# RQLuo/CDLNet-video

Measured on AMD Instinct MI355X. Metric: Mpix/s denoised (fwd+bwd) at K=30,M=64,P=7, higher is better.
Workload: dtype f32 (split-bf16 x3 MFMA, fp32 accumulate, fp32 storage)

## Files before the change

### cdlnet-video_amd/csrc/cdl_fused2d.hip

```cpp
#include <atomic>
#include <cstdlib>
#include <type_traits>
#include <mutex>
#include <utility>
#include <vector>

#include "cdl_common.h"
#include "cdl_fused_sweep.h"


namespace {

#include "cdl_wave_dev.h"

typedef __attribute__((ext_vector_type(4))) __bf16 bf16x4;

constexpr int WX = 2;
constexpr int RB = 8;
constexpr int TW = 32 * WX;
constexpr int HALO = 3;
constexpr int RTW = TW + 2 * HALO;
constexpr int RTC = RTW + 2;
constexpr int LDS_W = 32 * 64 * 16;
constexpr int LDS_TAU = 64 * 4;

constexpr int GW_TH = 16;
constexpr int GW_RTH = GW_TH + 2 * HALO;
constexpr int TROWS = GW_RTH + 1;
constexpr int TPITCH = 72;
constexpr int TCOPY = TROWS * TPITCH;
constexpr int WG_THIN_BYTES = 2 * 2 * 4 * TCOPY * 2;
constexpr int IMG_ELEMS = 32 * 32;

template <int WY_>
struct Shape {
    static_assert(WY_ == 2 || WY_ == 4, "64 x 16 or 64 x 32 tiles");
    static constexpr int WY = WY_;
    static constexpr int NW = WX * WY;
    static constexpr int NT = 64 * NW;
    static constexpr int TH = RB * WY;
    static constexpr int RTH = TH + 2 * HALO;
    static constexpr int PITCH = WY == 2 ? 28 : 44;
    static constexpr int COPY = RTC * PITCH;
    static constexpr int LDS_RT = 2 * 4 * COPY * 2;
    static constexpr int SLAB = RTH * RTW;
    static constexpr int LDS_RSUM = 4 * SLAB * 4;
    static constexpr int LDS_TACC = NW * 64 * 4;
    static constexpr int LDS_STAGE = LDS_RT + LDS_RSUM + LDS_W + LDS_TAU + LDS_TACC;
    static constexpr int LDS_DA_THIN = 2 * 4 * TCOPY * 2;
    static constexpr int LDS_DA = LDS_DA_THIN + NW * 2 * 2 * IMG_ELEMS * 2;
    static constexpr bool WREG = WY == 2;
};

struct FusedParams {
    const float *r;
    const float *zin;
    unsigned *map;
    float *zout;
    const float *tau;
    float *dtau;
    const uint4 *frags;
    float *patches;
    float sgn;
    int do_synth;
    CDL_DBG_FIELD(int dbg;)
    int N, H, W, tilesX, tilesY;
    int rev;
    const float *r2;
    float *da_partial;
    int drop_zout;
};
struct FusedMapParams : FusedParams {
    const float *cmap;
    const float *tslope;
    float *dtau_w;
    float *dcmap;
    int dc_add;
};

constexpr int MODE_MAP = 4, MODE_FWD_MAP = MODE_FWD | MODE_MAP, MODE_FIRST_MAP = MODE_FIRST | MODE_MAP, MODE_BWD_MAP = MODE_BWD | MODE_MAP;
template <int MODE_M> using StageParams = std::conditional_t<(MODE_M & MODE_MAP) != 0, FusedMapParams, FusedParams>;

__device__ __forceinline__ float embed7(const float *w, int P, int i, int j)
{
    const int off = (7 - P) / 2;
    const int ii = i - off, jj = j - off;
    if (i > 6 || j > 6 || ii < 0 || jj < 0 || ii >= P || jj >= P) return 0.0f;
    return w[ii * P + jj];
}

__device__ __forceinline__ void prep_one(const float *__restrict__ wA, const float *__restrict__ wB,
                                         uint4 *__restrict__ out, int MT, int P, int t)
{
    const int FA = MT * 4, FB = 4 * MT;
    if (t >= (FA + FB) * 64) return;
    const int lane = t & 63, f = t >> 6;
    const int row = lane & 31, h = lane >> 5;
    const int PP = P * P;
    float v[8];
    if (f < FA) {
        const int R = f / 4, ks = f % 4;
        const int ch = 32 * R + row;
#pragma unroll
        for (int jj = 0; jj < 8; ++jj) v[jj] = embed7(wA + (size_t)ch * PP, P, jj, 2 * ks + h);
    } else {
        const int g = f - FA;
        const int Rp = g / (2 * MT), ksB = g % (2 * MT);
        const int R = ksB >> 1, s = ksB & 1;
        const int tap = 32 * Rp + row;
#pragma unroll
        for (int jj = 0; jj < 8; ++jj) {
            const int ch = 32 * R + 16 * s + 8 * (jj >> 2) + 4 * h + (jj & 3);
            v[jj] = embed7(wB + (size_t)ch * PP, P, tap >> 3, tap & 7);
        }
    }
    bf16x8 hi, lo;
#pragma unroll
    for (int jj = 0; jj < 8; ++jj) {
        __bf16 hh, ll;
        split_bf16(v[jj], hh, ll);
        hi[jj] = hh;
        lo[jj] = ll;
    }
    uint4 *hi_dst, *lo_dst;
    if (f < FA) { hi_dst = out + (size_t)f * 64; lo_dst = out + (size_t)(FA + f) * 64; }
    else { hi_dst = out + (size_t)(2 * FA + (f - FA)) * 64; lo_dst = out + (size_t)(2 * FA + FB + (f - FA)) * 64; }
    hi_dst[lane] = __builtin_bit_cast(uint4, hi);
    lo_dst[lane] = __builtin_bit_cast(uint4, lo);
}

__global__ void k_prep(const float *__restrict__ wA, const float *__restrict__ wB,
                       uint4 *__restrict__ out, int MT, int P)
{
    prep_one(wA, wB, out, MT, P, blockIdx.x * blockDim.x + threadIdx.x);
}

constexpr int PREP_BATCH = 32;
struct PrepBatch {
    const float *wA[PREP_BATCH];
    const float *wB[PREP_BATCH];
};
__global__ void k_prep_batch(PrepBatch b, uint4 *__restrict__ out, int frag_uint4, int MT, int P)
{
    prep_one(b.wA[blockIdx.y], b.wB[blockIdx.y], out + (size_t)blockIdx.y * frag_uint4, MT, P,
             blockIdx.x * blockDim.x + threadIdx.x);
}

#ifndef CDL_POL_STAGE_FAT_LD
#define CDL_POL_STAGE_FAT_LD 2
#endif
#ifndef CDL_POL_STAGE_FAT_ST
#define CDL_POL_STAGE_FAT_ST 0
#endif
#ifndef CDL_POL_WGRAD_FAT_LD
#define CDL_POL_WGRAD_FAT_LD 2
#endif
struct CachePolicy {
    static constexpr int stage_fat_ld = CDL_POL_STAGE_FAT_LD;
    static constexpr int stage_fat_st = CDL_POL_STAGE_FAT_ST;
    static constexpr int wgrad_fat_ld = CDL_POL_WGRAD_FAT_LD;
    static constexpr int narrow = 0;
};
__device__ __forceinline__ __amdgpu_buffer_rsrc_t fat_rsrc(const float *base, size_t img_floats)
{
    return __builtin_amdgcn_make_buffer_rsrc(const_cast<float *>(base), 0, (int)(img_floats * 4), 0x00020000);
}
__device__ __forceinline__ float buf_ld(__amdgpu_buffer_rsrc_t r, int voff, int soff)
{
    return __builtin_bit_cast(float, __builtin_amdgcn_raw_buffer_load_b32(r, voff, soff, CachePolicy::narrow));
}
__device__ __forceinline__ void buf_st(float v, __amdgpu_buffer_rsrc_t r, int voff, int soff)
{
    __builtin_amdgcn_raw_buffer_store_b32(__builtin_bit_cast(unsigned, v), r, voff, soff, CachePolicy::narrow);
}

enum { LAY_NCHW = 0, LAY_BLK = 1, LAY_BLK16 = 2 };
typedef __attribute__((ext_vector_type(2))) unsigned u32x2;

__host__ __device__ inline size_t blk_image_elems(int M, int H, int W) { return (size_t)H * ((W + 31) / 32) * M * 32; }
template <int LAY> __host__ __device__ inline size_t lay_image_bytes(int M, int H, int W)
{
    return LAY == LAY_NCHW ? (size_t)M * H * W * 4 : blk_image_elems(M, H, W) * (LAY == LAY_BLK ? 4 : 2);
}


__device__ __forceinline__ float bf16_round(float v) { return (float)(__bf16)v; }

template <int MT>
__device__ __forceinline__ void blk16_load_raw(u32x2 (&z)[MT][4], __amdgpu_buffer_rsrc_t rs, int voff)
{
#pragma unroll
    for (int R = 0; R < MT; ++R)
#pragma unroll
        for (int q = 0; q < 4; ++q)
            z[R][q] = __builtin_bit_cast(u32x2, __builtin_amdgcn_raw_buffer_load_b64(rs, voff, (8 * R + 2 * q) * 32 * 8, CachePolicy::narrow));
}
__device__ __forceinline__ float blk16_decode(const u32x2 &u, int e)
{
    const unsigned w = (e & 2) ? u.y : u.x;
    return __builtin_bit_cast(float, (e & 1) ? (w & 0xffff0000u) : (w << 16));
}

template <int LAY, int MT, int POL>
__device__ __forceinline__ void blk_load(float (&z)[MT][16], __amdgpu_buffer_rsrc_t rs, int voff)
{
    constexpr int EB = LAY == LAY_BLK ? 16 : 8;
#pragma unroll
    for (int R = 0; R < MT; ++R)
#pragma unroll
        for (int q = 0; q < 4; ++q) {
            const int soff = (8 * R + 2 * q) * 32 * EB;
            if constexpr (LAY == LAY_BLK) {
                typedef __attribute__((ext_vector_type(4))) float f32x4;
                const f32x4 f = __builtin_bit_cast(f32x4, __builtin_amdgcn_raw_buffer_load_b128(rs, voff, soff, POL));
                z[R][4 * q + 0] = f.x; z[R][4 * q + 1] = f.y; z[R][4 * q + 2] = f.z; z[R][4 * q + 3] = f.w;
            } else {
                const u32x2 u = __builtin_bit_cast(u32x2, __builtin_amdgcn_raw_buffer_load_b64(rs, voff, soff, CachePolicy::narrow));
                z[R][4 * q + 0] = __builtin_bit_cast(float, u.x << 16);
                z[R][4 * q + 1] = __builtin_bit_cast(float, u.x & 0xffff0000u);
                z[R][4 * q + 2] = __builtin_bit_cast(float, u.y << 16);
                z[R][4 * q + 3] = __builtin_bit_cast(float, u.y & 0xffff0000u);
            }
        }
}
template <int LAY, int POL>
__device__ __forceinline__ void blk_store4(float a0, float a1, float a2, float a3, __amdgpu_buffer_rsrc_t rs, int voff, int quad_pair)
{
    constexpr int EB = LAY == LAY_BLK ? 16 : 8;
    const int soff = quad_pair * 32 * EB;
    if constexpr (LAY == LAY_BLK) {
        typedef __attribute__((ext_vector_type(4))) float f32x4;
        const f32x4 f = {a0, a1, a2, a3};
        __builtin_amdgcn_raw_buffer_store_b128(__builtin_bit_cast(u32x4, f), rs, voff + soff, 0, POL);
    } else {
        u32x2 u;
        u.x = (__builtin_bit_cast(unsigned, a0) >> 16) | (__builtin_bit_cast(unsigned, a1) & 0xffff0000u);
        u.y = (__builtin_bit_cast(unsigned, a2) >> 16) | (__builtin_bit_cast(unsigned, a3) & 0xffff0000u);
        __builtin_amdgcn_raw_buffer_store_b64(u, rs, voff, soff, CachePolicy::narrow);
    }
}

template <int N>
__device__ __forceinline__ float lane_transpose_sum(const float (&v)[N], int c)
{
    float r = LaneTransposeSum<N>::run(v, c);
    if (N == 16) r += __shfl_xor(r, 16, 64);
    return r;
}

__device__ __forceinline__ float col2im_row(const float (&rv)[4], int h)
{
    const float r4 = upper_half_to_lower(rv[0]);
    const float r5 = upper_half_to_lower(rv[1]);
    const float r6 = upper_half_to_lower(rv[2]);
    const bool lo = h == 0;
    float s = lo ? r6 : 0.0f;
    s = wave_shr1(s) + (lo ? r5 : 0.0f);
    s = wave_shr1(s) + (lo ? r4 : 0.0f);
    s = wave_shr1(s) + (lo ? rv[3] : 0.0f);
    s = wave_shr1(s) + (lo ? rv[2] : 0.0f);
    s = wave_shr1(s) + (lo ? rv[1] : 0.0f);
    s = wave_shr1(s) + (lo ? rv[0] : 0.0f);
    return s;
}

constexpr int RUN = 8;
typedef __attribute__((ext_vector_type(2))) __bf16 bf16x2;
template <int S>
__device__ __forceinline__ void store_run(__bf16 *dst, const __bf16 (&v)[RUN], bool low)
{
    static_assert(S >= 0 && S <= 3, "four shifted copies");
    if (!low) {
        if constexpr (S == 1) dst[-1] = v[0];
        if constexpr (S == 2) *reinterpret_cast<bf16x2 *>(dst - 2) = bf16x2{v[0], v[1]};
        if constexpr (S == 3) { dst[-3] = v[0]; *reinterpret_cast<bf16x2 *>(dst - 2) = bf16x2{v[1], v[2]}; }
    }
    *reinterpret_cast<bf16x4 *>(dst) = bf16x4{v[S], v[S + 1], v[S + 2], v[S + 3]};
    if constexpr (S == 0) *reinterpret_cast<bf16x4 *>(dst + 4) = bf16x4{v[4], v[5], v[6], v[7]};
    if constexpr (S == 1) { *reinterpret_cast<bf16x2 *>(dst + 4) = bf16x2{v[5], v[6]}; dst[6] = v[7]; }
    if constexpr (S == 2) *reinterpret_cast<bf16x2 *>(dst + 4) = bf16x2{v[6], v[7]};
    if constexpr (S == 3) dst[4] = v[7];
}
template <int PREC>
__device__ __forceinline__ void store_run_copies(__bf16 *dst, int copy_elems, const float (&f)[RUN], bool low)
{
    __bf16 hh[RUN], ll[RUN];
#pragma unroll
    for (int j = 0; j < RUN; ++j) split_bf16(f[j], hh[j], ll[j]);
    store_run<0>(dst, hh, low); store_run<1>(dst + copy_elems, hh, low);
    store_run<2>(dst + 2 * copy_elems, hh, low); store_run<3>(dst + 3 * copy_elems, hh, low);
    if (PREC != 1) {
        dst += 4 * copy_elems;
        store_run<0>(dst, ll, low); store_run<1>(dst + copy_elems, ll, low);
        store_run<2>(dst + 2 * copy_elems, ll, low); store_run<3>(dst + 3 * copy_elems, ll, low);
    }
}


struct TileAt { int tile, n, tyi, txi; };
__device__ __forceinline__ TileAt tile_decode(int t, int numTiles, int tilesX, int tilesY, int rev)
{
    TileAt q;
    q.tile = rev ? numTiles - 1 - t : t;
    int bid = q.tile;
    q.txi = bid % tilesX; bid /= tilesX;
    q.tyi = bid % tilesY;
    q.n = bid / tilesY;
    return q;
}

__device__ __forceinline__ bf16x8 lds_window8(const __bf16 *p)
{
    const bf16x4 a0 = *reinterpret_cast<const bf16x4 *>(p);
    const bf16x4 a1 = *reinterpret_cast<const bf16x4 *>(p + 4);
    return __builtin_shufflevector(a0, a1, 0, 1, 2, 3, 4, 5, 6, 7);
}

template <int N>
__device__ __forceinline__ void zero_tiles(f32x16 (&a)[N])
{
#pragma unroll
    for (int i = 0; i < N; ++i)
#pragma unroll
        for (int v = 0; v < 16; ++v) a[i][v] = 0.0f;
}

__device__ __forceinline__ float4 lane_channel_quad(const float *src, int R, int qv, int h)
{
    return *reinterpret_cast<const float4 *>(&src[32 * R + 8 * qv + 4 * h]);
}
template <int MT>
__device__ __forceinline__ void lane_channel_values(float (&out)[MT * 16], const float *src, int h)
{
#pragma unroll
    for (int R = 0; R < MT; ++R)
#pragma unroll
        for (int qv = 0; qv < 4; ++qv) {
            const float4 s4 = lane_channel_quad(src, R, qv, h);
            out[16 * R + 4 * qv + 0] = s4.x; out[16 * R + 4 * qv + 1] = s4.y;
            out[16 * R + 4 * qv + 2] = s4.z; out[16 * R + 4 * qv + 3] = s4.w;
        }
}

template <bool ALO>
__device__ __forceinline__ void wgrad_transpose_store(__bf16 *img, int qv, int c, int h, bf16x4 hi4, bf16x4 lo4)
{
    const int slot = (2 * qv + h) ^ ((c >> 1) & 7);
    __bf16 *dst = img + c * 32 + slot * 4;
    *reinterpret_cast<bf16x4 *>(dst) = hi4;
    if (ALO) *reinterpret_cast<bf16x4 *>(dst + IMG_ELEMS) = lo4;
}
template <bool ALO>
__device__ __forceinline__ void wgrad_transpose_store(__bf16 *img, int qv, int c, int h, float v0, float v1, float v2, float v3)
{
    const float val[4] = {v0, v1, v2, v3};
    bf16x4 hi4, lo4;
#pragma unroll
    for (int e = 0; e < 4; ++e) {
        __bf16 hh, ll;
        split_bf16(val[e], hh, ll);
        hi4[e] = hh;
        lo4[e] = ll;
    }
    wgrad_transpose_store<ALO>(img, qv, c, h, hi4, lo4);
}

template <int MT, int PREC, bool ALO>
__device__ __forceinline__ void wgrad_products(f32x16 (&acc)[MT][2], const __bf16 *wimg, const __bf16 *thin_hi, int yl,
                                               int wxi, int lane)
{
    const int c = lane & 31, h = lane >> 5;
#pragma unroll
    for (int kk = 0; kk < 2; ++kk) {
        bf16x8 Bh[2], Bl[2];
#pragma unroll
        for (int tt = 0; tt < 2; ++tt) {
            const int tap = 32 * tt + c, ti = tap >> 3, tj = tap & 7;
            const int e0 = wxi * 32 + 16 * kk + 8 * h + (tj & 4);
            const __bf16 *ph = thin_hi + (tj & 3) * TCOPY + (yl + ti) * TPITCH + e0;
            Bh[tt] = lds_window8(ph);
            if (PREC != 1) Bl[tt] = lds_window8(ph + 4 * TCOPY);
        }
#pragma unroll
        for (int R = 0; R < MT; ++R) {
            const int gg = (lane >> 4) & 1, qq = (lane >> 2) & 3, pp = lane & 3;
            bf16x4 part[2][2];
#pragma unroll
            for (int half = 0; half < 2; ++half) {
                const int row = 16 * kk + 8 * h + 4 * half + qq;
                const int slot = (4 * gg + pp) ^ ((row >> 1) & 7);
                const __bf16 *src = wimg + (size_t)(R * 2) * IMG_ELEMS + row * 32 + slot * 4;
                part[0][half] = __builtin_amdgcn_ds_read_tr16_b64_v4bf16(
                    (__attribute__((address_space(3))) bf16x4 *)(src));
                if (ALO)
                    part[1][half] = __builtin_amdgcn_ds_read_tr16_b64_v4bf16(
                        (__attribute__((address_space(3))) bf16x4 *)(src + IMG_ELEMS));
            }
            const bf16x8 Ah = __builtin_shufflevector(part[0][0], part[0][1], 0, 1, 2, 3, 4, 5, 6, 7);
// ... 56 lines not shown
    constexpr bool MAP = (MODE_M & MODE_MAP) != 0;
    using G = Shape<WY>;
    constexpr int NW = G::NW, NT = G::NT, TH = G::TH, RTH = G::RTH, PITCH = G::PITCH, COPY = G::COPY, SLAB = G::SLAB;
    constexpr int LDS_RT = G::LDS_RT, LDS_RSUM = G::LDS_RSUM, LDS_STAGE = G::LDS_STAGE, LDS_DA_THIN = G::LDS_DA_THIN;
    static_assert(!DA || (MODE == MODE_BWD && TH == GW_TH), "dA_k rides in the reverse stage, on k_wgrad2d's 64 x 16 tiles");
    extern __shared__ __attribute__((aligned(16))) unsigned char smem[];
    __bf16 *rt = reinterpret_cast<__bf16 *>(smem);
    float *rsum_all = reinterpret_cast<float *>(smem + LDS_RT);
    const uint4 *wl = reinterpret_cast<const uint4 *>(smem + LDS_RT + LDS_RSUM);
    float *tau_s = reinterpret_cast<float *>(smem + LDS_RT + LDS_RSUM + LDS_W);
    float *tacc_s = tau_s + 64;
    __bf16 *thin2 = reinterpret_cast<__bf16 *>(smem + LDS_STAGE);
    __bf16 *imgs2 = reinterpret_cast<__bf16 *>(smem + LDS_STAGE + LDS_DA_THIN);
    float *slope_s = MODE == MODE_BWD ? tau_s : tacc_s;
    float *tacc_w_s = reinterpret_cast<float *>(smem + LDS_STAGE + (DA ? G::LDS_DA : 0));

    constexpr int M = 32 * MT;
    constexpr int FA = MT * 4, FB = 4 * MT;
    constexpr int NFRAG = (PREC != 1 ? 2 : 1) * (FA + FB);
    const int tid = threadIdx.x, lane = tid & 63, wid = tid >> 6;
    const int wxi = wid % WX, wyi = wid / WX;
    const int c = lane & 31, h = lane >> 5;
    const size_t HW = (size_t)p.H * p.W;
    const int numTiles = p.N * p.tilesY * p.tilesX;

    {
        uint4 *z4 = reinterpret_cast<uint4 *>(smem);
        for (int i = tid; i < (LDS_RT + LDS_RSUM) / 16; i += NT) z4[i] = make_uint4(0, 0, 0, 0);
        uint4 *wdst = reinterpret_cast<uint4 *>(smem + LDS_RT + LDS_RSUM);
        if (PREC != 1) {
            for (int i = tid; i < NFRAG * 64; i += NT) wdst[i] = p.frags[i];
        } else {
            for (int i = tid; i < FA * 64; i += NT) wdst[i] = p.frags[i];
            for (int i = tid; i < FB * 64; i += NT) wdst[FA * 64 + i] = p.frags[2 * FA * 64 + i];
        }
        if constexpr (MAP) {
            if (tid < M) slope_s[tid] = p.tslope[tid];
        }
    }
    constexpr int RT_RUNS = (RTH + RUN - 1) / RUN;
    static_assert(RTW * RT_RUNS <= NT && RT_RUNS * RUN <= PITCH, "one run per thread; a column's runs stay inside its pitch");
    const int rt_xx = tid % RTW, rt_y0 = (tid / RTW) * RUN;
    const bool rt_on = tid < RTW * RT_RUNS;
    __bf16 *const rt_dst = rt + rt_xx * PITCH + rt_y0;
    float stg[RUN];
    auto stage_load = [&](int t) {
        const TileAt q = tile_decode(t, numTiles, p.tilesX, p.tilesY, p.rev);
        const float *rimg = p.r + (size_t)q.n * HW;
        const int gy0 = q.tyi * TH - HALO + rt_y0, gx = q.txi * TW - HALO + rt_xx;
        const bool colok = rt_on && t < numTiles && !CDL_DBG(p.dbg, 8) && gx >= 0 && gx < p.W;
#pragma unroll
        for (int j = 0; j < RUN; ++j) {
            const int gy = gy0 + j;
            float v = 0.0f;
            if (colok && rt_y0 + j < RTH && gy >= 0 && gy < p.H) v = rimg[(size_t)gy * p.W + gx];
            stg[j] = v;
        }
    };
    auto stage_store = [&]() {
        if (rt_on) store_run_copies<PREC>(rt_dst, COPY, stg, rt_y0 == 0);
    };
    constexpr int T2_RUNS = (RTW + RUN - 1) / RUN;
    static_assert(!DA || (GW_RTH * T2_RUNS <= NT && T2_RUNS * RUN <= TPITCH), "one run per thread; a row's runs stay inside its pitch");
    const int t2_x0 = (tid % T2_RUNS) * RUN, t2_yy = tid / T2_RUNS;
    const bool t2_on = tid < GW_RTH * T2_RUNS;
    __bf16 *const t2_dst = thin2 + t2_yy * TPITCH + t2_x0;
    float stg2[DA ? RUN : 1];
    auto stage2_load = [&](int t) {
        const TileAt q = tile_decode(t, numTiles, p.tilesX, p.tilesY, p.rev);
        const float *timg = p.r2 + (t < numTiles ? (size_t)q.n * HW : 0);
        const int gy = q.tyi * TH - HALO + t2_yy, gx0 = q.txi * TW - HALO + t2_x0;
        const bool rowok = t2_on && t < numTiles && !CDL_DBG(p.dbg, 8) && gy >= 0 && gy < p.H;
#pragma unroll
        for (int j = 0; j < (DA ? RUN : 1); ++j) {
            const int gx = gx0 + j;
            const bool ok = rowok && t2_x0 + j < RTW && gx >= 0 && gx < p.W;
            const float v = timg[ok ? (size_t)gy * p.W + gx : 0];
            stg2[j] = ok ? v : 0.0f;
        }
    };
    auto stage2_store = [&]() {
        if constexpr (DA) {
            if (t2_on) store_run_copies<PREC>(t2_dst, TCOPY, stg2, t2_x0 == 0);
        }
    };
    f32x16 dacc[DA ? MT : 1][2];
    if constexpr (DA) {
#pragma unroll
        for (int R = 0; R < MT; ++R) zero_tiles(dacc[R]);
        for (int i = tid; i < LDS_DA_THIN / 16; i += NT) reinterpret_cast<uint4 *>(thin2)[i] = make_uint4(0, 0, 0, 0);
        stage2_load(blockIdx.x);
    }
    stage_load(blockIdx.x);
    __syncthreads();
    stage_store();
    if constexpr (DA) stage2_store();

    constexpr int OFF_AH = 0;
    constexpr int OFF_AL = FA;
    constexpr int OFF_BH = (PREC != 1 ? 2 * FA : FA);
    constexpr int OFF_BL = 2 * FA + FB;
    constexpr bool WREG = G::WREG;
    bf16x8 wreg[WREG ? NFRAG : 1];
    if constexpr (WREG) {
#pragma unroll
        for (int f = 0; f < NFRAG; ++f) wreg[f] = __builtin_bit_cast(bf16x8, wl[f * 64 + lane]);
    }
    auto wfrag = [&](int f) __attribute__((always_inline)) {
        if constexpr (WREG) return wreg[f];
        else return __builtin_bit_cast(bf16x8, wl[f * 64 + lane]);
    };

    constexpr bool MAP_FWD = MAP && MODE != MODE_BWD;
    float tslr[MAP_FWD ? MT * 16 : 1];
    bool slope_any = false;
    if constexpr (MAP_FWD) {
        lane_channel_values<MT>(tslr, slope_s, h);
        slope_any = __ballot(lane < M && !(slope_s[lane] >= 0.0f && slope_s[lane] < __builtin_inff())) != 0ull;
    }

    const int xl = wxi * 32 + c;
    float *rsum = rsum_all + ((wxi & 1) + 2 * (wyi & 1)) * SLAB;
    const bool has_base = (MODE == MODE_FWD) || (MODE == MODE_BWD && p.zin != nullptr);
    const int hw4 = (int)HW * 4;

#pragma unroll 1
    for (int t = blockIdx.x; t < numTiles; t += gridDim.x) {
    const TileAt at = tile_decode(t, numTiles, p.tilesX, p.tilesY, p.rev);
    const int tile = at.tile, n = at.n;
    const int tx0 = at.txi * TW, ty0 = at.tyi * TH;
    const int x = tx0 + xl;
    if (MODE != MODE_BWD && tid < M) tau_s[tid] = p.tau[(size_t)n * M + tid];
    __syncthreads();
    constexpr bool LOAD_AHEAD = MODE != MODE_BWD || WY == 2;
    if (LOAD_AHEAD) {
        stage_load(t + gridDim.x);
        if constexpr (DA) stage2_load(t + gridDim.x);
    }

    float ring[7][4];
#pragma unroll
    for (int i = 0; i < 7; ++i)
#pragma unroll
        for (int j = 0; j < 4; ++j) ring[i][j] = 0.0f;
    float tsum[MT * 16];
#pragma unroll
    for (int i = 0; i < MT * 16; ++i) tsum[i] = 0.0f;
    constexpr bool MAP_BWD = MAP && MODE == MODE_BWD;
    float tsum_w[MAP_BWD ? MT * 16 : 1];
    if constexpr (MAP_BWD) {
#pragma unroll
        for (int i = 0; i < MT * 16; ++i) tsum_w[i] = 0.0f;
    }
    const bool tau_neg = (MODE != MODE_BWD && __ballot(lane < M && !(tau_s[lane] >= 0.0f)) != 0ull) || slope_any;
    float taur[MT * 16];
    if (MODE != MODE_BWD) lane_channel_values<MT>(taur, tau_s, h);

    const bool xok = x < p.W;
    const size_t img_in = lay_image_bytes<LIN>(M, p.H, p.W), img_out = lay_image_bytes<LOUT>(M, p.H, p.W);
    const __amdgpu_buffer_rsrc_t rs_in = uniform_rsrc(
        has_base ? (const char *)p.zin + (size_t)n * img_in : (const char *)p.zout, has_base ? img_in : 0);
    unsigned *const map_n = p.map ? p.map + ((size_t)n * 4 + 2 * h) * HW : nullptr;
    const __amdgpu_buffer_rsrc_t rs_out = uniform_rsrc((const char *)p.zout + (size_t)n * img_out, img_out);
    const int lane_off = (int)((4 * h) * HW + x) * 4;
    const int XB = (p.W + 31) / 32, xb = (tx0 >> 5) + wxi;
    constexpr int EB_IN = LIN == LAY_BLK16 ? 8 : 16, EB_OUT = LOUT == LAY_BLK16 ? 8 : 16;
    const int lane_blk_in = (h * 32 + c) * EB_IN, lane_blk_out = (h * 32 + c) * EB_OUT;

#pragma unroll 1
    for (int b = 0; b < RB; ++b) {
        const int yl = wyi * RB + b;
        const int y = ty0 + yl;
        const bool valid = xok && (y < p.H);
        const int voff = valid ? lane_off + y * p.W * 4 : OOB;
        const int blk = (y * XB + xb) * (M / 4) * 32;
        const int voff_in = LIN == LAY_NCHW ? voff : (valid ? blk * EB_IN + lane_blk_in : OOB);
        const int voff_st = (CDL_DBG(p.dbg, 1) || (MODE == MODE_BWD && p.drop_zout)) ? OOB : (LOUT == LAY_NCHW ? voff : (valid ? blk * EB_OUT + lane_blk_out : OOB));

        float zc[MT][16];
        u32x2 zr[MT][4];
        if (MODE != MODE_FIRST && LIN == LAY_BLK16) {
            blk16_load_raw<MT>(zr, rs_in, voff_in);
        } else if (MODE != MODE_FIRST && CDL_DBG(p.dbg, 16)) {
#pragma unroll
            for (int R = 0; R < MT; ++R)
#pragma unroll
                for (int v = 0; v < 16; ++v) zc[R][v] = 0.25f;
        } else if (MODE != MODE_FIRST && LIN != LAY_NCHW) {
            blk_load<LIN, MT, CachePolicy::stage_fat_ld>(zc, rs_in, voff_in);
        } else if (MODE != MODE_FIRST) {
#pragma unroll
            for (int R = 0; R < MT; ++R)
#pragma unroll
                for (int v = 0; v < 16; ++v) {
                    const int soff = (32 * R + 8 * (v >> 2) + (v & 3)) * hw4;
                    zc[R][v] = buf_ld(rs_in, voff, soff);
                }
        }
        unsigned sup = 0, sgb = 0;
        if (MODE == MODE_BWD && valid) {
            sup = map_n[(size_t)y * p.W + x];
            sgb = map_n[HW + (size_t)y * p.W + x];
        }
        float cm = 0.0f;
        if constexpr (MAP) {
            if (valid) cm = p.cmap[(size_t)n * HW + (size_t)y * p.W + x];
        }

        const int q = b & 3, e = yl - q;
        bf16x8 rh[4], rl[4];
#pragma unroll
        for (int ks = 0; ks < 4; ++ks) {
            const int col = xl + 2 * ks + h;
            rh[ks] = lds_window8(rt + (0 * 4 + q) * COPY + col * PITCH + e);
            if (PREC != 1) rl[ks] = lds_window8(rt + (1 * 4 + q) * COPY + col * PITCH + e);
        }

        __builtin_amdgcn_sched_barrier(0);
        f32x16 acc[MT];
        zero_tiles(acc);
        if CDL_DBG(p.dbg, 4) {
#pragma unroll
            for (int R = 0; R < MT; ++R) acc[R][0] = (float)rh[0][0] + (float)rl[1][1];
        } else {
            bf16x8 wh[2][MT], wlo[2][MT];
#pragma unroll
            for (int R = 0; R < MT; ++R) {
                wh[0][R] = wfrag(OFF_AH + R * 4);
                if (PREC != 1) wlo[0][R] = wfrag(OFF_AL + R * 4);
            }
#pragma unroll
            for (int ks = 0; ks < 4; ++ks) {
                const int cu = ks & 1, nx = cu ^ 1;
                if (ks + 1 < 4) {
#pragma unroll
                    for (int R = 0; R < MT; ++R) {
                        wh[nx][R] = wfrag(OFF_AH + R * 4 + ks + 1);
                        if (PREC != 1) wlo[nx][R] = wfrag(OFF_AL + R * 4 + ks + 1);
                    }
                }
                if (PREC != 1) {
#pragma unroll
                    for (int R = 0; R < MT; ++R) acc[R] = __builtin_amdgcn_mfma_f32_32x32x16_bf16(wlo[cu][R], rh[ks], acc[R], 0, 0, 0);
#pragma unroll
                    for (int R = 0; R < MT; ++R) acc[R] = __builtin_amdgcn_mfma_f32_32x32x16_bf16(wh[cu][R], rl[ks], acc[R], 0, 0, 0);
                    if (PREC == 2) {
#pragma unroll
                        for (int R = 0; R < MT; ++R) acc[R] = __builtin_amdgcn_mfma_f32_32x32x16_bf16(wlo[cu][R], rl[ks], acc[R], 0, 0, 0);
                    }
                }
#pragma unroll
                for (int R = 0; R < MT; ++R) acc[R] = __builtin_amdgcn_mfma_f32_32x32x16_bf16(wh[cu][R], rh[ks], acc[R], 0, 0, 0);
            }
        }

        __builtin_amdgcn_sched_barrier(0);
        auto epilogue = [&](auto general_shrink) {
#pragma unroll
        for (int R = 0; R < MT; ++R)
#pragma unroll
            for (int v = 0; v < 16; ++v) {
                const int chl = 32 * R + 8 * (v >> 2) + (v & 3);
                float zz;
                float zbase = 0.0f;
                if (MODE != MODE_FIRST) zbase = LIN == LAY_BLK16 ? blk16_decode(zr[R][v >> 2], v & 3) : zc[R][v];
                if (MODE == MODE_BWD) {
                    const bool on = (sup >> (16 * R + v)) & 1u;
                    zz = on ? zbase + acc[R][v] : 0.0f;
                    const float gt = ((sgb >> (16 * R + v)) & 1u) ? zz : -zz;
                    tsum[16 * R + v] += gt;
                    if constexpr (MAP_BWD) tsum_w[16 * R + v] = fmaf(cm, gt, tsum_w[16 * R + v]);
                } else {
                    const float base = (MODE == MODE_FWD) ? zbase : 0.0f;
                    const float u = fmaf(p.sgn, acc[R][v], base);
                    float tt = taur[16 * R + v];
                    if constexpr (MAP_FWD) tt = cdl_map_threshold(tt, cm, tslr[16 * R + v]);
                    const float st = decltype(general_shrink)::value ? cdl_shrink(u, tt)
                                                                     : u - __builtin_amdgcn_fmed3f(u, -tt, tt);
                    zz = CDL_DBG(p.dbg, 64) ? u : (valid ? st : 0.0f);
                }
                if (LOUT == LAY_BLK16) zz = bf16_round(zz);
                if (LOUT == LAY_NCHW) buf_st(zz, rs_out, voff_st, chl * hw4);
                acc[R][v] = zz;
            }
        };
        bool general = tau_neg;
        if constexpr (MAP_FWD) general = general || __ballot(!(cm >= 0.0f && cm < __builtin_inff())) != 0ull;
        if (general) epilogue(std::true_type{});
        else epilogue(std::false_type{});
        if (LOUT != LAY_NCHW) {
#pragma unroll
            for (int R = 0; R < MT; ++R)
#pragma unroll
                for (int q = 0; q < 4; ++q)
                    blk_store4<LOUT, CachePolicy::stage_fat_st>(acc[R][4 * q], acc[R][4 * q + 1], acc[R][4 * q + 2], acc[R][4 * q + 3], rs_out,
                                     voff_st, 8 * R + 2 * q);
        }
        if (MODE != MODE_BWD && map_n) {
            unsigned ws = 0, wg = 0;
#pragma unroll
            for (int R = 0; R < MT; ++R)
#pragma unroll
                for (int v = 0; v < 16; ++v) {
                    const float zz = acc[R][v];
                    ws |= (zz != 0.0f ? 1u : 0u) << (16 * R + v);
                    wg |= (__builtin_bit_cast(unsigned, zz) >> 31) << (16 * R + v);
                }
            if (valid && !CDL_DBG(p.dbg, 1)) {
                map_n[(size_t)y * p.W + x] = ws;
                map_n[HW + (size_t)y * p.W + x] = wg;
            }
        }
        if constexpr (MAP_BWD) {
            if (p.dcmap) {
                float dcs = 0.0f;
#pragma unroll
                for (int R = 0; R < MT; ++R)
#pragma unroll
                    for (int qv = 0; qv < 4; ++qv) {
                        const float4 s4 = lane_channel_quad(slope_s, R, qv, h);
                        const float sl[4] = {s4.x, s4.y, s4.z, s4.w};
#pragma unroll
                        for (int e = 0; e < 4; ++e) {
                            const int v = 4 * qv + e;
                            const float zz = acc[R][v];
                            dcs = fmaf(sl[e], ((sgb >> (16 * R + v)) & 1u) ? zz : -zz, dcs);
                        }
                    }
                dcs += __shfl_xor(dcs, 32, 64);
                if (h == 0 && valid) {
                    float *dst = p.dcmap + (size_t)n * HW + (size_t)y * p.W + x;
                    *dst = p.dc_add ? *dst + dcs : dcs;
                }
            }
        }
        if constexpr (DA) {
            __bf16 *wimg = imgs2 + (size_t)wid * (MT * 2) * IMG_ELEMS;
            constexpr bool ALO = PREC != 1 && LOUT != LAY_BLK16;
#pragma unroll
            for (int R = 0; R < MT; ++R)
#pragma unroll
                for (int qv = 0; qv < 4; ++qv)
                    wgrad_transpose_store<ALO>(wimg + (size_t)(R * 2) * IMG_ELEMS, qv, c, h, acc[R][4 * qv], acc[R][4 * qv + 1],
                                               acc[R][4 * qv + 2], acc[R][4 * qv + 3]);
            __builtin_amdgcn_fence(__ATOMIC_RELEASE, "wavefront");
            __builtin_amdgcn_wave_barrier();
            wgrad_products<MT, PREC, ALO>(dacc, wimg, thin2, yl, wxi, lane);
        }
        if (MODE == MODE_BWD && !p.do_synth) continue;
        if CDL_DBG(p.dbg, 2) { ring[0][0] += acc[0][0] + acc[MT - 1][15]; continue; }

        __builtin_amdgcn_sched_barrier(0);
        f32x16 D[2];
        zero_tiles(D);
        {
            bf16x8 bwh[2][2], bwl[2][2];
#pragma unroll
            for (int Rp = 0; Rp < 2; ++Rp) {
                bwh[0][Rp] = wfrag(OFF_BH + Rp * 2 * MT);
                if (PREC != 1) bwl[0][Rp] = wfrag(OFF_BL + Rp * 2 * MT);
            }
#pragma unroll
            for (int q = 0; q < 2 * MT; ++q) {
                const int R = q >> 1, s = q & 1, cu = q & 1, nx = cu ^ 1;
                if (q + 1 < 2 * MT) {
#pragma unroll
                    for (int Rp = 0; Rp < 2; ++Rp) {
                        bwh[nx][Rp] = wfrag(OFF_BH + Rp * 2 * MT + q + 1);
                        if (PREC != 1) bwl[nx][Rp] = wfrag(OFF_BL + Rp * 2 * MT + q + 1);
                    }
                }
                bf16x8 zh, zl;
#pragma unroll
                for (int jj = 0; jj < 8; ++jj) {
                    __bf16 hh, ll;
                    split_bf16(acc[R][8 * s + jj], hh, ll);
                    zh[jj] = hh;
                    if (PREC != 1 && LOUT != LAY_BLK16) zl[jj] = ll;
                }
                if (PREC != 1) {
#pragma unroll
                    for (int Rp = 0; Rp < 2; ++Rp) D[Rp] = __builtin_amdgcn_mfma_f32_32x32x16_bf16(bwl[cu][Rp], zh, D[Rp], 0, 0, 0);
                    if (LOUT != LAY_BLK16) {
#pragma unroll
                        for (int Rp = 0; Rp < 2; ++Rp) D[Rp] = __builtin_amdgcn_mfma_f32_32x32x16_bf16(bwh[cu][Rp], zl, D[Rp], 0, 0, 0);
                        if (PREC == 2) {
#pragma unroll
                            for (int Rp = 0; Rp < 2; ++Rp) D[Rp] = __builtin_amdgcn_mfma_f32_32x32x16_bf16(bwl[cu][Rp], zl, D[Rp], 0, 0, 0);
                        }
                    }
                }
#pragma unroll
                for (int Rp = 0; Rp < 2; ++Rp) D[Rp] = __builtin_amdgcn_mfma_f32_32x32x16_bf16(bwh[cu][Rp], zh, D[Rp], 0, 0, 0);
            }
        }

        __builtin_amdgcn_sched_barrier(0);
#pragma unroll
        for (int Rp = 0; Rp < 2; ++Rp)
#pragma unroll
            for (int v = 0; v < 16; ++v) {
                const int i = 4 * Rp + (v >> 2);
                if (i <= 6) ring[i][v & 3] += D[Rp][v];
            }
        {
            const float cs = col2im_row(ring[0], h);
            if (lane < 38 && !CDL_DBG(p.dbg, 32)) rsum[yl * RTW + 32 * wxi + lane] = cs;
        }
#pragma unroll
        for (int i = 0; i < 6; ++i)
#pragma unroll
            for (int jl = 0; jl < 4; ++jl) ring[i][jl] = ring[i + 1][jl];
#pragma unroll
        for (int jl = 0; jl < 4; ++jl) ring[6][jl] = 0.0f;
    }

    if (MODE != MODE_BWD || p.do_synth) {
#pragma unroll
        for (int i = 0; i < 6; ++i) {
            const float cs = col2im_row(ring[i], h);
            if (lane < 38 && !CDL_DBG(p.dbg, 32)) rsum[(wyi * RB + RB + i) * RTW + 32 * wxi + lane] = cs;
        }
    }
    if (MODE == MODE_BWD) {
        tsum_to_lds<MT>(tsum, tacc_s + wid * 64, c, h);
        if constexpr (MAP_BWD) tsum_to_lds<MT>(tsum_w, tacc_w_s + wid * 64, c, h);
    }
    __syncthreads();
    if (!LOAD_AHEAD) stage_load(t + gridDim.x);
    if (MODE == MODE_BWD && tid < M) {
        float sacc = 0.0f;
#pragma unroll
        for (int w = 0; w < NW; ++w) sacc += tacc_s[w * 64 + tid];
        p.dtau[(size_t)tile * M + tid] = sacc;
        if constexpr (MAP_BWD) {
            float saccw = 0.0f;
#pragma unroll
            for (int w = 0; w < NW; ++w) saccw += tacc_w_s[w * 64 + tid];
            p.dtau_w[(size_t)tile * M + tid] = saccw;
        }
    }
    if CDL_DBG(p.dbg, 128) continue;
    if (MODE != MODE_BWD || p.do_synth) {
        typedef __attribute__((ext_vector_type(4))) float f32x4;
        using PV = std::conditional_t<WY == 2, f32x4, float>;
        constexpr int NV = SLAB * 4 / (int)sizeof(PV);
        static_assert(SLAB * 4 % sizeof(PV) == 0 && LDS_RT % sizeof(PV) == 0, "slabs and patches are whole vectors");
        PV *patch = reinterpret_cast<PV *>(p.patches + (size_t)tile * SLAB);
        PV *rs = reinterpret_cast<PV *>(rsum_all);
        for (int i = tid; i < NV; i += NT) {
            patch[i] = (rs[i] + rs[NV + i]) + (rs[2 * NV + i] + rs[3 * NV + i]);
            rs[i] = (PV)(0.0f); rs[NV + i] = (PV)(0.0f); rs[2 * NV + i] = (PV)(0.0f); rs[3 * NV + i] = (PV)(0.0f);
        }
    }
    stage_store();
    if constexpr (DA) stage2_store();
    }
    if constexpr (DA) {
        float *red = reinterpret_cast<float *>(smem);
        wgrad_wave_sum<MT, NW, 1>(dacc, red, 0, wid, tid, p.da_partial + (size_t)blockIdx.x * 2 * M * 64);
    }
}

template <int WY>
__device__ __forceinline__ float patch_sum(const float *__restrict__ patches, int n, int Y, int X,
                                           int tilesX, int tilesY)
{
    constexpr int TH = Shape<WY>::TH, SLAB = Shape<WY>::SLAB;
    const int tyc = Y / TH, txc = X / TW;
    const int ly = Y - tyc * TH, lx = X - txc * TW;
    const int hx = (lx < HALO && txc > 0) ? -1 : ((lx >= TW - HALO && txc + 1 < tilesX) ? 1 : 0);
    const int vy = (ly < HALO && tyc > 0) ? -1 : ((ly >= TH - HALO && tyc + 1 < tilesY) ? 1 : 0);
    const float *own = patches + (((size_t)n * tilesY + tyc) * tilesX + txc) * SLAB + (ly + HALO) * RTW + lx + HALO;
    const ptrdiff_t dx = (ptrdiff_t)hx * (SLAB - TW), dy = (ptrdiff_t)vy * ((ptrdiff_t)tilesX * SLAB - TH * RTW);
    float sum = 0.0f;
    if (vy < 0) {
        if (hx < 0) sum += own[dy + dx];
        sum += own[dy];
        if (hx > 0) sum += own[dy + dx];
    }
    if (hx < 0) sum += own[dx];
    sum += own[0];
    if (hx > 0) sum += own[dx];
    if (vy > 0) {
        if (hx < 0) sum += own[dy + dx];
        sum += own[dy];
        if (hx > 0) sum += own[dy + dx];
    }
    return sum;
}

template <int ASM_ROWS, int WY>
__global__ __launch_bounds__(256) void k_assemble(const float *__restrict__ patches,
                                                  const float *__restrict__ mask,
                                                  const float *__restrict__ sub, float alpha,
                                                  float *__restrict__ out, int N, int H, int W,
                                                  int tilesX, int tilesY, float *__restrict__ acc, int acc_add)
{
    const int X = blockIdx.x * 256 + threadIdx.x, n = blockIdx.z;
    if (X >= W) return;
#pragma unroll
    for (int j = 0; j < ASM_ROWS; ++j) {
        const int Y = blockIdx.y * ASM_ROWS + j;
        if (Y >= H) break;
        const size_t i = ((size_t)n * H + Y) * W + X;
        const float raw = patch_sum<WY>(patches, n, Y, X, tilesX, tilesY);
        if (acc) acc[i] = acc_add ? acc[i] + raw : raw;
        if (!out) continue;
        float sum = alpha * raw;
        if (mask) sum *= mask[i];
        if (sub) sum -= sub[i];
        out[i] = sum;
    }
}

template <int WY>
__global__ __launch_bounds__(256) void k_assemble_v4(const float *__restrict__ patches,
                                                     const float *__restrict__ mask, const float *__restrict__ sub,
                                                     float alpha, float *__restrict__ out, int N, int H, int W,
                                                     int tilesX, int tilesY, float *__restrict__ accum, int acc_add)
{
    constexpr int TH = Shape<WY>::TH, SLAB = Shape<WY>::SLAB;
    const int X = (blockIdx.x * 64 + (threadIdx.x & 63)) * 4, n = blockIdx.z;
    if (X >= W) return;
    const int txc = X / TW, lx = X - txc * TW;
    int hx[4];
#pragma unroll
    for (int e = 0; e < 4; ++e)
        hx[e] = (lx + e < HALO && txc > 0) ? -1 : ((lx + e >= TW - HALO && txc + 1 < tilesX) ? 1 : 0);
#pragma unroll
    for (int j = 0; j < 2; ++j) {
        const int Y = (blockIdx.y * 4 + (threadIdx.x >> 6)) * 2 + j;
        if (Y >= H) break;
        const int tyc = Y / TH, ly = Y - tyc * TH;
        const int vy = (ly < HALO && tyc > 0) ? -1 : ((ly >= TH - HALO && tyc + 1 < tilesY) ? 1 : 0);
        const float *own = patches + (((size_t)n * tilesY + tyc) * tilesX + txc) * SLAB + (ly + HALO) * RTW + lx + HALO;
        const ptrdiff_t dy = (ptrdiff_t)vy * ((ptrdiff_t)tilesX * SLAB - TH * RTW);
        float acc[4] = {0.0f, 0.0f, 0.0f, 0.0f};
        auto row = [&](ptrdiff_t off) {
            float a[4], b[4];
#pragma unroll
            for (int e = 0; e < 4; ++e) {
                a[e] = own[off + e];
                b[e] = hx[e] != 0 ? own[off + e + (ptrdiff_t)hx[e] * (SLAB - TW)] : 0.0f;
            }
#pragma unroll
            for (int e = 0; e < 4; ++e) {
                if (hx[e] < 0) acc[e] += b[e];
                acc[e] += a[e];
                if (hx[e] > 0) acc[e] += b[e];
            }
        };
        if (vy < 0) row(dy);
        row(0);
        if (vy > 0) row(dy);
        const size_t i = ((size_t)n * H + Y) * W + X;
        if (accum) {
            float4 a = make_float4(acc[0], acc[1], acc[2], acc[3]);
            if (acc_add) {
                const float4 o = *reinterpret_cast<const float4 *>(accum + i);
                a.x += o.x; a.y += o.y; a.z += o.z; a.w += o.w;
            }
            *reinterpret_cast<float4 *>(accum + i) = a;
        }
        if (!out) continue;
        float4 v = make_float4(alpha * acc[0], alpha * acc[1], alpha * acc[2], alpha * acc[3]);
        if (mask) {
            const float4 m = *reinterpret_cast<const float4 *>(mask + i);
            v.x *= m.x; v.y *= m.y; v.z *= m.z; v.w *= m.w;
        }
        if (sub) {
            const float4 sv = *reinterpret_cast<const float4 *>(sub + i);
            v.x -= sv.x; v.y -= sv.y; v.z -= sv.z; v.w -= sv.w;
        }
        *reinterpret_cast<float4 *>(out + i) = v;
    }
}
// ... 913 lines not shown
```

### cdlnet-video_amd/csrc/cdl_wave_dev.h

```cpp
#pragma once

typedef __attribute__((ext_vector_type(8))) __bf16 bf16x8;
typedef __attribute__((ext_vector_type(16))) float f32x16;
typedef __attribute__((ext_vector_type(4))) unsigned u32x4;

constexpr int OOB = 0x7fff0000;

enum { MODE_FWD = 0, MODE_FIRST = 1, MODE_BWD = 2 };

template <bool SCALAR_SIZE = false>
__device__ __forceinline__ __amdgpu_buffer_rsrc_t uniform_rsrc(const void *base, size_t bytes)
{
    const unsigned long long a = reinterpret_cast<unsigned long long>(base);
    const unsigned lo = __builtin_amdgcn_readfirstlane((unsigned)a);
    const unsigned hi = __builtin_amdgcn_readfirstlane((unsigned)(a >> 32));
    void *b = reinterpret_cast<void *>(((unsigned long long)hi << 32) | lo);
    return __builtin_amdgcn_make_buffer_rsrc(b, 0, SCALAR_SIZE ? (int)bytes : __builtin_amdgcn_readfirstlane((int)bytes), 0x00020000);
}

__device__ __forceinline__ void split_bf16(float v, __bf16 &hi, __bf16 &lo)
{
    hi = (__bf16)v;
    lo = (__bf16)(v - (float)hi);
}
__device__ __forceinline__ void split_bf16(const float (&v)[8], bf16x8 &hi, bf16x8 &lo)
{
#pragma unroll
    for (int i = 0; i < 8; ++i) {
        __bf16 h, l;
        split_bf16(v[i], h, l);
        hi[i] = h;
        lo[i] = l;
    }
}

__device__ __forceinline__ void mfma_split3(f32x16 &acc, const bf16x8 &ah, const bf16x8 &al, const bf16x8 &bh, const bf16x8 &bl)
{
    acc = __builtin_amdgcn_mfma_f32_32x32x16_bf16(al, bh, acc, 0, 0, 0);
    acc = __builtin_amdgcn_mfma_f32_32x32x16_bf16(ah, bl, acc, 0, 0, 0);
    acc = __builtin_amdgcn_mfma_f32_32x32x16_bf16(ah, bh, acc, 0, 0, 0);
}

template <int P> __host__ __device__ constexpr int tap_slot(int i, int j)
{
    if (P == 5) return (i < 4 && j < 4) ? 8 * i + j : (i < 4 ? 8 * i + 4 : (j < 4 ? 8 * j + 5 : 6));
    return 8 * i + j;
}
template <int P> struct TapTiles { static constexpr int RT = (P == 7) ? 2 : 1; };

__device__ __forceinline__ float wave_shr1(float v)
{
    return __builtin_bit_cast(float, __builtin_amdgcn_update_dpp(0, __builtin_bit_cast(int, v), 0x138, 0xf, 0xf, true));
}
__device__ __forceinline__ float upper_half_to_lower(float v)
{
    float lo = 0.0f;
    asm volatile("s_nop 1\n\tv_permlane32_swap_b32 %0, %1\n\ts_nop 1" : "+v"(v), "+v"(lo));
    return lo;
}

template <int N>
struct LaneTransposeSum {
    static __device__ __forceinline__ float run(const float (&v)[N], int c)
    {
        constexpr int n = N / 2;
        const bool up = (c & n) != 0;
        float w[n];
#pragma unroll
        for (int k = 0; k < n; ++k) {
            const float keep = up ? v[k + n] : v[k];
            const float send = up ? v[k] : v[k + n];
            w[k] = keep + __shfl_xor(send, n, 64);
        }
        return LaneTransposeSum<n>::run(w, c);
    }
};
template <>
struct LaneTransposeSum<1> {
    static __device__ __forceinline__ float run(const float (&v)[1], int) { return v[0]; }
};
```

Measured before the change: 126.5.

## Prefetch next row's stage loads, defer tsum accumulation, use DPP for lane transpose

In backward mode the per-row z/map/cmap loads are now issued one row ahead, into registers that persist across iterations, so their latency overlaps the current row's MFMA work. The tau-gradient sign-flip accumulation moves out of the MFMA epilogue into the split/synthesis loop (shadowed), and it uses a branchless XOR sign flip. Lane-transpose reductions within 16-lane rows switch from ds_bpermute shuffles to DPP moves. The trade-off is higher register pressure from the prefetch buffers, which could lower occupancy or cause spills.

```diff
diff --git a/cdlnet-video_amd/csrc/cdl_fused2d.hip b/cdlnet-video_amd/csrc/cdl_fused2d.hip
--- a/cdlnet-video_amd/csrc/cdl_fused2d.hip
+++ b/cdlnet-video_amd/csrc/cdl_fused2d.hip
@@ -155,6 +155,15 @@
 #ifndef CDL_POL_WGRAD_FAT_LD
 #define CDL_POL_WGRAD_FAT_LD 2
 #endif
+#ifndef CDL_STAGE_TSUM_SHADOW
+#define CDL_STAGE_TSUM_SHADOW 1
+#endif
+#ifndef CDL_STAGE_TSUM_DPP
+#define CDL_STAGE_TSUM_DPP 1
+#endif
+#ifndef CDL_STAGE_PREFETCH
+#define CDL_STAGE_PREFETCH 1
+#endif
 struct CachePolicy {
     static constexpr int stage_fat_ld = CDL_POL_STAGE_FAT_LD;
     static constexpr int stage_fat_st = CDL_POL_STAGE_FAT_ST;
@@ -240,10 +249,17 @@
     }
 }
 
+template <bool FIRST, class A, class B>
+__device__ __forceinline__ decltype(auto) pick_ref(A &a, B &b)
+{
+    if constexpr (FIRST) return (a);
+    else return (b);
+}
+
 template <int N>
 __device__ __forceinline__ float lane_transpose_sum(const float (&v)[N], int c)
 {
-    float r = LaneTransposeSum<N>::run(v, c);
+    float r = LaneTransposeSum<N, CDL_STAGE_TSUM_DPP != 0>::run(v, c);
     if (N == 16) r += __shfl_xor(r, 16, 64);
     return r;
 }
@@ -606,6 +622,14 @@
 #pragma unroll
         for (int i = 0; i < MT * 16; ++i) tsum_w[i] = 0.0f;
     }
+    constexpr bool TS_SHADOW = CDL_STAGE_TSUM_SHADOW && MODE == MODE_BWD && LOUT != LAY_BLK16 && !MAP;
+    auto tsum_add = [&](int R, int v, float zz, unsigned sgb, float cm) __attribute__((always_inline)) {
+        if CDL_DBG(p.dbg, 256) return;
+        const unsigned flip = (~sgb << (31 - (16 * R + v))) & 0x80000000u;
+        const float gt = __builtin_bit_cast(float, __builtin_bit_cast(unsigned, zz) ^ flip);
+        tsum[16 * R + v] += gt;
+        if constexpr (MAP_BWD) tsum_w[16 * R + v] = fmaf(cm, gt, tsum_w[16 * R + v]);
+    };
     const bool tau_neg = (MODE != MODE_BWD && __ballot(lane < M && !(tau_s[lane] >= 0.0f)) != 0ull) || slope_any;
     float taur[MT * 16];
     if (MODE != MODE_BWD) lane_channel_values<MT>(taur, tau_s, h);
@@ -621,6 +645,52 @@
     constexpr int EB_IN = LIN == LAY_BLK16 ? 8 : 16, EB_OUT = LOUT == LAY_BLK16 ? 8 : 16;
     const int lane_blk_in = (h * 32 + c) * EB_IN, lane_blk_out = (h * 32 + c) * EB_OUT;
 
+    auto fat_loads = [&](int y, bool valid, int voff, int voff_in, float (&zc)[MT][16], u32x2 (&zr)[MT][4], unsigned &sup,
+                         unsigned &sgb, float &cm) __attribute__((always_inline)) {
+        if (MODE != MODE_FIRST && LIN == LAY_BLK16) {
+            blk16_load_raw<MT>(zr, rs_in, voff_in);
+        } else if (MODE != MODE_FIRST && CDL_DBG(p.dbg, 16)) {
+#pragma unroll
+            for (int R = 0; R < MT; ++R)
+#pragma unroll
+                for (int v = 0; v < 16; ++v) zc[R][v] = 0.25f;
+        } else if (MODE != MODE_FIRST && LIN != LAY_NCHW) {
+            blk_load<LIN, MT, CachePolicy::stage_fat_ld>(zc, rs_in, voff_in);
+        } else if (MODE != MODE_FIRST) {
+#pragma unroll
+            for (int R = 0; R < MT; ++R)
+#pragma unroll
+                for (int v = 0; v < 16; ++v) {
+                    const int soff = (32 * R + 8 * (v >> 2) + (v & 3)) * hw4;
+                    zc[R][v] = buf_ld(rs_in, voff, soff);
+                }
+        }
+        sup = 0; sgb = 0;
+        if (MODE == MODE_BWD && valid) {
+            sup = map_n[(size_t)y * p.W + x];
+            sgb = map_n[HW + (size_t)y * p.W + x];
+        }
+        cm = 0.0f;
+        if constexpr (MAP) {
+            if (valid) cm = p.cmap[(size_t)n * HW + (size_t)y * p.W + x];
+        }
+    };
+    constexpr bool PREFETCH = CDL_STAGE_PREFETCH && MODE == MODE_BWD && WY == 2;
+    float zc_a[PREFETCH ? MT : 1][PREFETCH ? 16 : 1];
+    u32x2 zr_a[PREFETCH ? MT : 1][PREFETCH ? 4 : 1];
+    unsigned sup_a = 0, sgb_a = 0;
+    float cm_a = 0.0f;
+    auto fat_loads_ahead = [&](int b_, bool live) __attribute__((always_inline)) {
+        if constexpr (PREFETCH) {
+            const int y = ty0 + wyi * RB + b_;
+            const bool valid = live && xok && (y < p.H);
+            const int voff = valid ? lane_off + y * p.W * 4 : OOB;
+            const int blk = (y * XB + xb) * (M / 4) * 32;
+            fat_loads(y, valid, voff, LIN == LAY_NCHW ? voff : (valid ? blk * EB_IN + lane_blk_in : OOB), zc_a, zr_a, sup_a, sgb_a, cm_a);
+        }
+    };
+    fat_loads_ahead(0, true);
+
 #pragma unroll 1
     for (int b = 0; b < RB; ++b) {
         const int yl = wyi * RB + b;
@@ -631,35 +701,15 @@
         const int voff_in = LIN == LAY_NCHW ? voff : (valid ? blk * EB_IN + lane_blk_in : OOB);
         const int voff_st = (CDL_DBG(p.dbg, 1) || (MODE == MODE_BWD && p.drop_zout)) ? OOB : (LOUT == LAY_NCHW ? voff : (valid ? blk * EB_OUT + lane_blk_out : OOB));
 
-        float zc[MT][16];
-        u32x2 zr[MT][4];
-        if (MODE != MODE_FIRST && LIN == LAY_BLK16) {
-            blk16_load_raw<MT>(zr, rs_in, voff_in);
-        } else if (MODE != MODE_FIRST && CDL_DBG(p.dbg, 16)) {
-#pragma unroll
-            for (int R = 0; R < MT; ++R)
-#pragma unroll
-                for (int v = 0; v < 16; ++v) zc[R][v] = 0.25f;
-        } else if (MODE != MODE_FIRST && LIN != LAY_NCHW) {
-            blk_load<LIN, MT, CachePolicy::stage_fat_ld>(zc, rs_in, voff_in);
-        } else if (MODE != MODE_FIRST) {
-#pragma unroll
-            for (int R = 0; R < MT; ++R)
-#pragma unroll
-                for (int v = 0; v < 16; ++v) {
-                    const int soff = (32 * R + 8 * (v >> 2) + (v & 3)) * hw4;
-                    zc[R][v] = buf_ld(rs_in, voff, soff);
-                }
-        }
-        unsigned sup = 0, sgb = 0;
-        if (MODE == MODE_BWD && valid) {
-            sup = map_n[(size_t)y * p.W + x];
-            sgb = map_n[HW + (size_t)y * p.W + x];
-        }
-        float cm = 0.0f;
-        if constexpr (MAP) {
-            if (valid) cm = p.cmap[(size_t)n * HW + (size_t)y * p.W + x];
-        }
+        float zc_b[PREFETCH ? 1 : MT][PREFETCH ? 1 : 16];
+        u32x2 zr_b[PREFETCH ? 1 : MT][PREFETCH ? 1 : 4];
+        unsigned sup_b = 0, sgb_b = 0;
+        float cm_b = 0.0f;
+        float (&zc)[MT][16] = pick_ref<PREFETCH>(zc_a, zc_b);
+        u32x2 (&zr)[MT][4] = pick_ref<PREFETCH>(zr_a, zr_b);
+        unsigned &sup = PREFETCH ? sup_a : sup_b, &sgb = PREFETCH ? sgb_a : sgb_b;
+        float &cm = PREFETCH ? cm_a : cm_b;
+        if constexpr (!PREFETCH) fat_loads(y, valid, voff, voff_in, zc, zr, sup, sgb, cm);
 
         const int q = b & 3, e = yl - q;
         bf16x8 rh[4], rl[4];
@@ -721,9 +771,7 @@
                 if (MODE == MODE_BWD) {
                     const bool on = (sup >> (16 * R + v)) & 1u;
                     zz = on ? zbase + acc[R][v] : 0.0f;
-                    const float gt = ((sgb >> (16 * R + v)) & 1u) ? zz : -zz;
-                    tsum[16 * R + v] += gt;
-                    if constexpr (MAP_BWD) tsum_w[16 * R + v] = fmaf(cm, gt, tsum_w[16 * R + v]);
+                    if constexpr (!TS_SHADOW) tsum_add(R, v, zz, sgb, cm);
                 } else {
                     const float base = (MODE == MODE_FWD) ? zbase : 0.0f;
                     const float u = fmaf(p.sgn, acc[R][v], base);
@@ -788,6 +836,12 @@
                 }
             }
         }
+        const unsigned sgb_t = sgb;
+        const float cm_t = cm;
+        if constexpr (PREFETCH) {
+            fat_loads_ahead(b + 1, b + 1 < RB);
+            __builtin_amdgcn_sched_barrier(0);
+        }
         if constexpr (DA) {
             __bf16 *wimg = imgs2 + (size_t)wid * (MT * 2) * IMG_ELEMS;
             constexpr bool ALO = PREC != 1 && LOUT != LAY_BLK16;
@@ -801,8 +855,16 @@
             __builtin_amdgcn_wave_barrier();
             wgrad_products<MT, PREC, ALO>(dacc, wimg, thin2, yl, wxi, lane);
         }
-        if (MODE == MODE_BWD && !p.do_synth) continue;
-        if CDL_DBG(p.dbg, 2) { ring[0][0] += acc[0][0] + acc[MT - 1][15]; continue; }
+        if ((MODE == MODE_BWD && !p.do_synth) || CDL_DBG(p.dbg, 2)) {
+            if constexpr (TS_SHADOW) {
+#pragma unroll
+                for (int R = 0; R < MT; ++R)
+#pragma unroll
+                    for (int v = 0; v < 16; ++v) tsum_add(R, v, acc[R][v], sgb_t, cm_t);
+            }
+            if CDL_DBG(p.dbg, 2) ring[0][0] += acc[0][0] + acc[MT - 1][15];
+            continue;
+        }
 
         __builtin_amdgcn_sched_barrier(0);
         f32x16 D[2];
@@ -831,6 +893,7 @@
                     split_bf16(acc[R][8 * s + jj], hh, ll);
                     zh[jj] = hh;
                     if (PREC != 1 && LOUT != LAY_BLK16) zl[jj] = ll;
+                    if constexpr (TS_SHADOW) tsum_add(R, 8 * s + jj, acc[R][8 * s + jj], sgb_t, cm_t);
                 }
                 if (PREC != 1) {
 #pragma unroll
@@ -876,7 +939,10 @@
             if (lane < 38 && !CDL_DBG(p.dbg, 32)) rsum[(wyi * RB + RB + i) * RTW + 32 * wxi + lane] = cs;
         }
     }
-    if (MODE == MODE_BWD) {
+    if (MODE == MODE_BWD && CDL_DBG(p.dbg, 256)) {
+        tacc_s[wid * 64 + lane] = 0.0f;
+        if constexpr (MAP_BWD) tacc_w_s[wid * 64 + lane] = 0.0f;
+    } else if (MODE == MODE_BWD) {
         tsum_to_lds<MT>(tsum, tacc_s + wid * 64, c, h);
         if constexpr (MAP_BWD) tsum_to_lds<MT>(tsum_w, tacc_w_s + wid * 64, c, h);
     }
diff --git a/cdlnet-video_amd/csrc/cdl_wave_dev.h b/cdlnet-video_amd/csrc/cdl_wave_dev.h
--- a/cdlnet-video_amd/csrc/cdl_wave_dev.h
+++ b/cdlnet-video_amd/csrc/cdl_wave_dev.h
@@ -59,7 +59,25 @@
     return lo;
 }
 
-template <int N>
+template <int DIST>
+__device__ __forceinline__ float lane_xor_dpp(float v)
+{
+    static_assert(DIST == 8 || DIST == 4 || DIST == 2 || DIST == 1, "distances inside a 16-lane row");
+    const int s = __builtin_bit_cast(int, v);
+    int r;
+    if constexpr (DIST == 8) {
+        r = __builtin_amdgcn_update_dpp(0, s, 0x128, 0xf, 0xf, false);
+    } else if constexpr (DIST == 4) {
+        r = __builtin_amdgcn_update_dpp(0, s, 0x104, 0xf, 0x5, false);
+        r = __builtin_amdgcn_update_dpp(r, s, 0x114, 0xf, 0xa, false);
+    } else if constexpr (DIST == 2) {
+        r = __builtin_amdgcn_update_dpp(0, s, 0x4e, 0xf, 0xf, false);
+    } else {
+        r = __builtin_amdgcn_update_dpp(0, s, 0xb1, 0xf, 0xf, false);
+    }
+    return __builtin_bit_cast(float, r);
+}
+template <int N, bool DPP = false>
 struct LaneTransposeSum {
     static __device__ __forceinline__ float run(const float (&v)[N], int c)
     {
@@ -70,12 +88,13 @@
         for (int k = 0; k < n; ++k) {
             const float keep = up ? v[k + n] : v[k];
             const float send = up ? v[k] : v[k + n];
-            w[k] = keep + __shfl_xor(send, n, 64);
+            if constexpr (DPP && n <= 8) w[k] = keep + lane_xor_dpp<n>(send);
+            else w[k] = keep + __shfl_xor(send, n, 64);
         }
-        return LaneTransposeSum<n>::run(w, c);
+        return LaneTransposeSum<n, DPP>::run(w, c);
     }
 };
-template <>
-struct LaneTransposeSum<1> {
+template <bool DPP>
+struct LaneTransposeSum<1, DPP> {
     static __device__ __forceinline__ float run(const float (&v)[1], int) { return v[0]; }
 };
```

Result: faster. 128.4, median of 6 (+1.5%).
